# Fabstir/fabstir-vectordb

Measured on AMD Instinct MI355X. Metric: k-NN queries/sec at recall@10>=0.95, 1Mx384 f32, higher is better.
Workload: dtype f32

## Files before the change

fabstir-vectordb_amd/csrc/fvdb_graph.cpp:

```cpp
#include <algorithm>
#include <chrono>
#include <cstdio>
#include <cstdlib>
#include <cstring>
#include <map>
#include <new>
#include <string>
#include <vector>

#include "fvdb_internal.h"
#include "common.h"
#include "kernels_graph.h"
#include "kernels_graph_fast.h"
#include "kernels_graph_build.h"
#include "kernels_graph_maint.h"

using namespace fvdb;

struct fvdb_graph {
  fvdb_store* store = nullptr;
  uint32_t M = 0, M0 = 0;
  uint32_t stride0 = 0, strideU = 0;
  uint32_t n = 0, n_cap = 0;
  uint32_t u_rows = 0, u_cap = 0;
// ... 871 lines not shown
  if (mask && mask->stamp != g->mutations) FAIL(ctx, FVDB_E_INVALID, "stale mask: the graph changed after the mask was created");
  if (on && on->device != s->ctx->device) FAIL(ctx, FVDB_E_INVALID, "context of another device");
  if (s->d != s->dpad && slot != 0) FAIL(ctx, FVDB_E_UNSUPPORTED, "padded dimensions use slot 0 only");
  if (!g->uploaded || !g->has_entry) FAIL(ctx, FVDB_E_INVALID, "graph not uploaded");
  if (k == 0 || ef == 0 || ef > 4096) FAIL(ctx, FVDB_E_UNSUPPORTED, "ef must be in 1..4096");
  if (B == 0) return FVDB_OK;
  HIPCHK(ctx, hipSetDevice(ctx->device));
  std::lock_guard<std::mutex> lk(g->mu);
  const float* qd = q_dev;
  if (s->d != s->dpad) {
    HIPCHK(ctx, g->s_q.ensure((size_t)B * s->dpad * 4));
    hipLaunchKernelGGL(graph_pad_rows_kernel, dim3(cdiv((uint64_t)B * s->dpad, 256)), dim3(256), 0, ctx->stream, q_dev, s->d,
                       s->dpad, (uint64_t)B, g->s_q.as<float>());
    qd = g->s_q.as<float>();
  }
  SearchPlan sp{};
  int rc;
  if ((rc = search_scratch(g, ctx, slot, B, ef, &sp)) || (rc = search_kernel(g, ctx, ef, &sp))) return rc;
  if (sp.lds > 48 * 1024)
    HIPCHK(ctx, hipFuncSetAttribute(sp.fast ? (const void*)sp.fast : (const void*)sp.exact, hipFuncAttributeMaxDynamicSharedMemorySize, (int)sp.lds));
  if (!g->d_counters.p) {
    HIPCHK(ctx, g->d_counters.ensure(32));
    HIPCHK(ctx, hipMemsetAsync(g->d_counters.p, 0, 32, ctx->stream));
  }
  const uint32_t* deleted = mask ? mask->flags.as<uint32_t>() : g->d_deleted.as<uint32_t>();
  const uint32_t any_deleted = mask ? 1u : (g->n_deleted ? 1u : 0u);
  const GraphView gv{s->data, g->d_level.as<uint32_t>(), deleted, g->d_adj0.as<uint32_t>(), g->d_ubase.as<uint32_t>(),
                     g->d_adjU.as<uint32_t>(), g->stride0, g->strideU, g->n, s->dpad, g->entry, g->top_level, any_deleted,
                     g->d_counters.as<unsigned long long>(), graph_stamps_report(g)};
  hipEvent_t* ev = nullptr;
  if (s->ctx->profiling) {
    ev = g->kev[g->kev_n & 63];
    if (!ev[0]) {
      (void)hipEventCreate(&ev[0]);
      (void)hipEventCreate(&ev[1]);
    }
    (void)hipEventRecord(ev[0], ctx->stream);
  }
  if (sp.fast)
    hipLaunchKernelGGL(sp.fast, dim3(cdiv(B, 4)), dim3(256), sp.lds, ctx->stream, gv, qd, B, k, ef, sp.cand_cap, sp.wave_lds,
                       g->s_visited[slot].as<uint8_t>(), sp.vstride, sp.words, g->s_touched[slot].as<uint32_t>(), sp.tcap, out_nodes_dev,
                       out_dist_dev, out_counts_dev, out_status_dev, (HItem*)g->s_spill[slot].p, sp.spill_cap);
  else
    hipLaunchKernelGGL(sp.exact, dim3(B), dim3(64), sp.lds, ctx->stream, gv, qd, B, k, ef, sp.cand_cap, g->s_visited[slot].as<uint32_t>(),
                       sp.vstride / 4, g->s_touched[slot].as<uint32_t>(), sp.tcap, out_nodes_dev, out_dist_dev, out_counts_dev,
                       out_status_dev, sp.rh ? (HItem*)g->s_spill[slot].p : nullptr, sp.rh ? sp.spill_cap : 0u);
// ... 333 lines not shown
```

fabstir-vectordb_amd/host/capi.cpp:

```cpp
#include <cstring>
#include <new>

#include "fvdb_host.hpp"

using namespace fvdbh;

extern "C" {

void* fvh_ivf_new(fvdb_ctx* ctx, uint32_t n_clusters, uint32_t n_probe, uint32_t train_size, uint32_t max_iterations,
                  uint64_t seed) {
  IVFConfig c;
  c.n_clusters = n_clusters;
  c.n_probe = n_probe;
  c.train_size = train_size;
  c.max_iterations = max_iterations;
  c.seed = seed;
  if (!c.is_valid()) return nullptr;
  return new (std::nothrow) IVFIndex(ctx, c);
}
void fvh_ivf_free(void* p) { delete (IVFIndex*)p; }
int fvh_ivf_train(void* p, const float* x, uint64_t n, uint32_t d, fvdb_train_result* out) {
  return ((IVFIndex*)p)->train(x, n, d, out);
}
int fvh_ivf_set_trained(void* p, const float* c, uint32_t d) { return ((IVFIndex*)p)->set_trained(c, d); }
// ... 302 lines not shown
uint64_t fvh_hnsw_vacuum(void* p) { return ((HNSWIndex*)p)->vacuum(); }
int fvh_hnsw_vacuum_ex(void* p, uint64_t* removed) { return ((HNSWIndex*)p)->vacuum(removed); }
void fvh_hnsw_set_resident_vacuum(void* p, int on) { ((HNSWIndex*)p)->set_resident_vacuum(on != 0); }
int fvh_hnsw_resident_vacuum(void* p) { return ((HNSWIndex*)p)->resident_vacuum(); }
void fvh_hnsw_set_vacuum_keep_rows(void* p, int on) { ((HNSWIndex*)p)->set_vacuum_keep_rows(on != 0); }
int fvh_hnsw_vacuum_info(void* p, fvdb_graph_maintenance_info_t* out) { return ((HNSWIndex*)p)->vacuum_info(out); }
uint64_t fvh_hnsw_store_rows(void* p) { return ((HNSWIndex*)p)->store_rows(); }
int fvh_hybrid_get_vectors(void* p, const uint64_t* ids, uint64_t n, float* out, uint8_t* found) {
  return ((HybridIndex*)p)->get_vectors(ids, n, out, found);
}
void fvh_hybrid_set_resident_migration(void* p, int on) { ((HybridIndex*)p)->set_resident_migration(on != 0); }
int fvh_hybrid_migration_info(void* p, fvdb_maintenance_info_t* out) { return ((HybridIndex*)p)->migration_info(out); }
uint64_t fvh_hybrid_timestamp_count(void* p) { return ((HybridIndex*)p)->timestamp_count(); }
void fvh_hybrid_export_timestamps(void* p, uint64_t* ids, double* ts) { ((HybridIndex*)p)->export_timestamps(ids, ts); }
uint64_t fvh_hybrid_recent_count(void* p) { return ((HybridIndex*)p)->recent_count(); }
uint64_t fvh_hybrid_historical_count(void* p) { return ((HybridIndex*)p)->historical_count(); }
int fvh_hybrid_is_initialized(void* p) { return ((HybridIndex*)p)->is_initialized(); }
int fvh_hybrid_is_ivf_trained(void* p) { return ((HybridIndex*)p)->is_ivf_trained(); }
void* fvh_hybrid_hnsw(void* p) { return &((HybridIndex*)p)->recent(); }
void fvh_hybrid_set_sequential_graph(void* p, int on) { ((HybridIndex*)p)->set_sequential_graph(on != 0); }
int fvh_hybrid_sequential_graph(void* p) { return ((HybridIndex*)p)->sequential_graph(); }
double fvh_hybrid_recent_build_seconds(void* p) { return ((HybridIndex*)p)->recent_build_seconds(); }
void fvh_hybrid_set_blocking_writers(void* p, int on) { ((HybridIndex*)p)->set_blocking_writers(on != 0); }
int fvh_hybrid_blocking_writers(void* p) { return ((HybridIndex*)p)->blocking_writers(); }
void* fvh_hybrid_ivf(void* p) { return &((HybridIndex*)p)->historical(); }

}
```

fabstir-vectordb_amd/host/fvdb_host.hpp:

```cpp
#pragma once
#include <atomic>
#include <condition_variable>
#include <cstdint>
#include <memory>
#include <mutex>
#include <shared_mutex>
#include <string>
#include <unordered_map>
#include <unordered_set>
#include <vector>

#include "../../include/fvdb.h"

namespace fvdbh {

struct SplitMix64 {
  uint64_t s;
  explicit SplitMix64(uint64_t seed) : s(seed) {}
  uint64_t next() {
    uint64_t z = (s += 0x9E3779B97F4A7C15ull);
    z = (z ^ (z >> 30)) * 0xBF58476D1CE4E5B9ull;
    z = (z ^ (z >> 27)) * 0x94D049BB133111EBull;
    return z ^ (z >> 31);
  }
// ... 41 lines not shown
  int reserve(fvdb_ctx* c, uint64_t bytes, bool pinned) {
    if (bytes <= cap) return FVDB_OK;
    release();
    ctx = c;
    if (fvdb_dev_alloc(c, bytes, &dev) || (pinned && fvdb_host_alloc(c, bytes, &host))) return FVDB_E_OOM;
    cap = bytes;
    return FVDB_OK;
  }
  void release() {
    if (dev) fvdb_dev_free(ctx, dev);
    if (host) fvdb_host_free(ctx, host);
    dev = host = nullptr;
    cap = 0;
  }
};

typedef std::shared_ptr<fvdb_mask> MaskRef;
inline MaskRef adopt_mask(fvdb_mask* m) { return MaskRef(m, [](fvdb_mask* p) { fvdb_mask_destroy(p); }); }
inline bool mask_fresh(const MaskRef& m) {
  fvdb_mask_info_t info;
  return m && fvdb_mask_info(m.get(), &info) == FVDB_OK && !info.stale;
}

inline int slot_ctx(fvdb_ctx* base, bool borrow, fvdb_ctx** ctx) {
  if (*ctx) return FVDB_OK;
  if (!borrow) return fvdb_ctx_create(fvdb_ctx_device(base), ctx);
  *ctx = base;
  return FVDB_OK;
}

struct IVFConfig {
  uint32_t n_clusters = 256, n_probe = 16, train_size = 10000, max_iterations = 25;
  uint64_t seed = 0;
  bool is_valid() const { return n_clusters > 0 && n_probe > 0 && n_probe <= n_clusters && train_size > 0 && max_iterations > 0; }
};

class IVFIndex {
 public:
  IVFIndex(fvdb_ctx* ctx, const IVFConfig& cfg);
  ~IVFIndex();
  const IVFConfig& config() const { return cfg_; }
  bool is_trained() const { return trained_; }
  uint32_t dimension() const { return dim_; }
  uint64_t total_vectors() const { return total_; }
  int train(const float* data, uint64_t n, uint32_t dim, fvdb_train_result* out);
  int set_trained(const float* centroids, uint32_t dim);
  int get_centroids(float* out) const;
  int insert(uint64_t id, const float* v, uint32_t dim);
  int batch_insert(const uint64_t* ids, const float* v, uint64_t n, uint32_t dim, uint64_t* n_ok, int* first_error);
  int batch_insert_assigned(const uint64_t* ids, const float* v, uint64_t n, uint32_t dim, const uint32_t* clusters,
                            uint64_t* n_ok, int* first_error);
  int batch_insert_from_store(const uint64_t* ids, fvdb_store* store, const uint32_t* rows, uint64_t n, uint64_t* n_ok,
// ... 83 lines not shown
  uint64_t node_count() const { return n_registered_; }
  bool entry_point(uint64_t* id) const;
  uint32_t dimension() const { return dim_; }
  size_t assign_level();
  int insert(uint64_t id, const float* v, uint32_t dim, int64_t forced_level);
  int batch_insert(const uint64_t* ids, const float* v, uint64_t n, uint32_t dim, const int64_t* levels, uint64_t* n_ok,
                   int* first_error);
  void set_device_insert(bool on, int mode = 0) {
    device_insert_ = on;
    insert_mode_ = mode;
  }
  bool device_insert() const { return device_insert_; }
  int set_insert_visited(int mode, uint32_t table_slots = 0);
  int insert_info(fvdb_graph_insert_info_t* out);
  const fvdb_graph_insert_stats& insert_stats() const { return insert_stats_; }
  uint64_t host_path_inserts() const { return n_host_inserts_; }
  uint64_t graph_upload_bytes() const { return graph_ ? fvdb_graph_upload_bytes(graph_) : 0; }
  fvdb_graph* device_graph() { return sync_graph() == FVDB_OK ? graph_ : nullptr; }
  int search(const float* q, uint32_t B, uint32_t dim, uint32_t k, uint32_t ef, uint64_t* ids, float* dist,
             uint32_t* counts);
  int search_dev(const float* q_dev, uint32_t B, uint32_t dim, uint32_t k, uint32_t ef, uint64_t* ids, float* dist,
                 uint32_t* counts);
  static constexpr uint32_t kSlots = 16;
  bool search_dev_begin(const float* q_dev, uint32_t B, uint32_t dim, uint32_t k, uint32_t ef, int* rc, uint32_t slot = 0,
                        const AllowView* view = nullptr);
  int search_dev_end(const float* q_dev, uint32_t B, uint32_t dim, uint32_t k, uint32_t ef, uint64_t* ids, float* dist,
                     uint32_t* counts, uint32_t slot = 0, const AllowView* view = nullptr);
  int allowed_view(const uint64_t* allowed, uint64_t n_allowed, ViewRef* out);
  int search_allowed(const float* q, uint32_t B, uint32_t dim, uint32_t k, uint32_t ef, const uint64_t* allowed,
                     uint64_t n_allowed, uint64_t* ids, float* dist, uint32_t* counts);
  int search_dev_view(const float* q_dev, uint32_t B, uint32_t dim, uint32_t k, uint32_t ef, const AllowView& view,
                      uint64_t* ids, float* dist, uint32_t* counts);
  void set_scan_cutoff(uint64_t nodes) { scan_cutoff_ = nodes; }
  uint64_t scan_cutoff() const { return scan_cutoff_; }
  bool scans(const AllowView& v, uint32_t k) const { return v.allowed_live <= scan_cutoff_ && k <= FVDB_MAX_K; }
  uint64_t mask_builds() const { return mask_builds_; }
  int mark_deleted(uint64_t id);
  bool is_deleted(uint64_t id) const;
  uint64_t active_count() const;
  int vacuum(uint64_t* removed);
  uint64_t vacuum() {
    uint64_t r = 0;
    return vacuum(&r) == FVDB_OK ? r : 0;
  }
  void set_resident_vacuum(bool on) { resident_vacuum_ = on; }
  bool resident_vacuum() const { return resident_vacuum_; }
// ... 76 lines not shown
  bool resident_vacuum_ = true, vacuum_keep_rows_ = false;
  int vacuum_path_ = VACUUM_NONE;
  fvdb_graph_maintenance_info_t vacuum_info_{};
  uint64_t vacuum_host(const std::vector<uint8_t>& dead, uint64_t removed);
  void vacuum_adopt(bool reclaimed, const std::vector<uint8_t>& dead);
  bool host_link_reported_ = false;
  fvdb_graph_insert_stats insert_stats_{};
  uint64_t n_host_inserts_ = 0;
  void add_insert_stats(const fvdb_graph_insert_stats& st);
  int ensure_graph_handle();
  int ensure_host_graph();
  bool device_insert_ok() const;
  int check_insert(uint64_t id, const float* v, uint32_t dim) const;
  int insert_host(uint64_t id, const float* v, uint32_t dim, int64_t forced_level);
  int append_nodes(const uint64_t* ids, const uint32_t* levels, const float* v, uint32_t m, uint32_t* first);
  template <class L>
  int adopt_nodes(const uint64_t* ids, const float* v, uint64_t n, uint32_t dim, const L* levels);
  int link_and_publish(uint32_t row, bool on_device);
  int link_host(uint32_t row, std::vector<std::pair<uint32_t, uint32_t>>* touched);
  void finalize_insert(uint32_t row);
  struct DevSlot {
    fvdb_ctx* ctx = nullptr;
    DevBuf buf;
  };
  DevSlot slots_[kSlots];
  DevBuf d_q_;
  std::atomic<uint64_t> n_fallback_{0};
  std::mutex sync_mu_, walk_mu_, search_mu_;
  uint64_t scan_cutoff_ = 8192;
  std::mutex view_mu_;
  std::vector<uint64_t> view_key_;
  ViewRef view_;
  uint64_t mask_builds_ = 0;

  fvdb_ctx* ctx_;
  HNSWConfig cfg_;
  SplitMix64 rng_;
  fvdb_store* store_ = nullptr;
  uint32_t dim_ = 0;
  bool has_dim_ = false, has_entry_ = false, entry_lost_ = false;
  uint32_t entry_ = 0;
  uint64_t n_registered_ = 0;
  std::vector<uint64_t> ids_;
  std::vector<uint32_t> level_;
  std::vector<uint8_t> deleted_, registered_;
  std::vector<std::vector<std::vector<uint32_t>>> nbrs_;
  std::unordered_map<uint64_t, uint32_t> index_of_;
  std::vector<float> host_vecs_;
// ... 20 lines not shown
struct HybridSearchConfig {
  bool search_recent = true, search_historical = true;
  uint64_t recent_k = 0, historical_k = 0;
  uint64_t k = 10, hnsw_ef = 50, ivf_n_probe = 10;
};

class HybridIndex {
 public:
  HybridIndex(fvdb_ctx* ctx_ivf, fvdb_ctx* ctx_hnsw, const HybridConfig& cfg);
  ~HybridIndex();
  bool is_initialized() const { return initialized_; }
  bool is_ivf_trained() const { return ivf_trained_; }
  int initialize(const float* data, uint64_t n, uint32_t dim);
  int set_ivf_centroids(const float* c, uint32_t dim);
  int insert_with_timestamp(uint64_t id, const float* v, uint32_t dim, double ts, double now, int64_t level);
  int search(const float* q, uint32_t B, uint32_t dim, const HybridSearchConfig& cfg, double now, uint64_t* ids,
             float* dist, uint32_t* counts);
  int search_dev(const float* q_dev, uint32_t B, uint32_t dim, const HybridSearchConfig& cfg, double now,
                 uint64_t* ids, float* dist, uint32_t* counts);
  static constexpr uint32_t kSlots = HNSWIndex::kSlots;
  int search_dev_begin(uint32_t slot, const float* q_dev, uint32_t B, uint32_t dim, const HybridSearchConfig& cfg,
                       double now);
  int search_dev_end(uint32_t slot, uint64_t* ids, float* dist, uint32_t* counts);
  int attach_comm(fvdb_comm* comm);
  int search_sharded_begin(uint32_t slot, const float* q_dev, uint32_t B, uint32_t dim, const HybridSearchConfig& cfg,
                           int mode, double now = 0.0);
  int search_sharded_end(uint32_t slot, uint64_t* ids, float* dist, uint32_t* counts) {
    return search_dev_end(slot, ids, dist, counts);
  }
  uint32_t sharded_rows(uint32_t B, int mode) const;
  typedef int (*FilterFn)(uint64_t id, void* user);
  int search_with_filter(const float* q, uint32_t B, uint32_t dim, uint64_t k, FilterFn matches, void* user, double now,
                         uint64_t* ids, float* dist, uint32_t* counts);
  int search_allowed(const float* q, uint32_t B, uint32_t dim, const HybridSearchConfig& cfg, const uint64_t* allowed,
                     uint64_t n_allowed, double now, uint64_t* ids, float* dist, uint32_t* counts);
  void set_blocking_writers(bool on) { writers_wait_ = on; }
  bool blocking_writers() const { return writers_wait_; }
  bool busy() const {
    std::lock_guard<std::mutex> lk(slot_mu_);
    for (const Slot& s : slots_)
      if (s.active) return true;
    return false;
  }
  bool migration_due(double threshold_s, double now) const {
    return !pending_migration_.empty() && age_of(now, pending_min_ts_) >= threshold_s;
  }
// ... 43 lines not shown
                 std::vector<uint64_t>& hid, std::vector<float>& hv);
  bool sequential_graph_ = true;
  bool resident_migration_ = true;
  int migration_path_ = MIGRATION_NONE;
  fvdb_maintenance_info_t migration_info_{};
  std::atomic<bool> writers_wait_{false};
  int write_lock(std::unique_lock<std::shared_mutex>& w);
  double recent_build_s_ = 0.0;
  fvdb_comm* comm_ = nullptr;
  fvdb_sharded* sharded_ = nullptr;
  uint32_t shard_rank_ = 0, shard_world_ = 0;
  std::vector<uint32_t> shard_owner_;
  std::vector<uint64_t> shard_sizes_;
  uint64_t migrate_locked(double threshold_s, double now);
  bool busy_unlocked() const {
    for (const Slot& s : slots_)
      if (s.active) return true;
    return false;
  }
  mutable std::shared_mutex rw_;
  mutable std::mutex slot_mu_;
  std::condition_variable slot_cv_;
  fvdb_ctx* ctx_ivf_;
  struct Slot {
    DevBuf ivf;
    uint32_t ivf_rows = 0;
    fvdb_event* ivf_done = nullptr;
    fvdb_ctx* ivf_ctx = nullptr;
    bool active = false, ivf_in_flight = false, hnsw_in_flight = false, recent = false;
    DevBuf d_q;
    const float* q = nullptr;
    uint32_t B = 0, dim = 0, k = 0, rk = 0, hk = 0, ef = 0;
    MaskRef ivf_mask;
    HNSWIndex::ViewRef view;
  };
  Slot slots_[kSlots];
  struct Lease {
    static constexpr uint32_t kAnyFree = ~0u;
    enum How { kTake, kAdopt };
    Lease(HybridIndex* h, uint32_t slot, How how);
    ~Lease();
    Lease(const Lease&) = delete;
    Lease& operator=(const Lease&) = delete;
    void hand_over() { sl = nullptr; }
    uint32_t index() const { return (uint32_t)(sl - h->slots_); }
    HybridIndex* h;
// ... 24 lines not shown
```

fabstir-vectordb_amd/host/hnsw_index.cpp:

```cpp
#include <omp.h>

#include <algorithm>
#include <chrono>
#include <cstdio>
#include <cstdlib>
#include <cstring>

#include "fvdb_host.hpp"

namespace fvdbh {

void RustHeap::sift_up(size_t start, size_t pos) {
  Cand elt = data[pos];
  while (pos > start) {
    size_t parent = (pos - 1) / 2;
    if (le(elt, data[parent])) break;
    data[pos] = data[parent];
    pos = parent;
  }
  data[pos] = elt;
}
void RustHeap::push(Cand c) {
  size_t old = data.size();
  data.push_back(c);
// ... 77 lines not shown
  long quota = -1, period = -1;
  if (FILE* f = fopen("/sys/fs/cgroup/cpu.max", "r")) {
    char q[64];
    if (fscanf(f, "%63s %ld", q, &period) == 2 && strcmp(q, "max") != 0) quota = atol(q);
    fclose(f);
  } else if (FILE* f1 = fopen("/sys/fs/cgroup/cpu/cpu.cfs_quota_us", "r")) {
    if (fscanf(f1, "%ld", &quota) != 1) quota = -1;
    fclose(f1);
    if (FILE* f2 = fopen("/sys/fs/cgroup/cpu/cpu.cfs_period_us", "r")) {
      if (fscanf(f2, "%ld", &period) != 1) period = -1;
      fclose(f2);
    }
  }
  if (quota > 0 && period > 0) n = std::min<long>(n, std::max<long>(1, (quota + period - 1) / period));
  return std::max(1, std::min(n, 64));
}

static inline bool set_insert(std::vector<uint32_t>& s, uint32_t v) {
  if (std::find(s.begin(), s.end(), v) != s.end()) return false;
  s.push_back(v);
  return true;
}

HNSWIndex::HNSWIndex(fvdb_ctx* ctx, const HNSWConfig& cfg) : ctx_(ctx), cfg_(cfg), rng_(cfg.seed) {}

HNSWIndex::~HNSWIndex() {
  view_.reset();
  if (graph_) fvdb_graph_destroy(graph_);
  for (uint32_t i = 0; i < kSlots; ++i) {
    slots_[i].buf.release();
    if (i > 0 && slots_[i].ctx) fvdb_ctx_destroy(slots_[i].ctx);
  }
  d_q_.release();
  for (Walk* w : {&search_walk_, &insert_walk_})
    if (w->sc) fvdb_scorer_destroy(w->sc);
  if (store_) fvdb_store_destroy(store_);
}

bool HNSWIndex::entry_point(uint64_t* id) const {
  if (!has_entry_) return false;
  *id = ids_[entry_];
  return true;
}

size_t HNSWIndex::assign_level() {
  size_t level = 0;
  while (rng_.gen_f64() < 0.408) level += 1;
  return level;
}

int HNSWIndex::ensure_store(uint32_t dim) {
  if (store_) return FVDB_OK;
  return fvdb_store_create(ctx_, dim, 1024, &store_);
}
// ... 247 lines not shown

namespace {
struct WalkBlock {
  uint32_t* nodes;
  float* dist;
  uint32_t *counts, *status;
  uint64_t bytes;
  WalkBlock(void* base, uint32_t B, uint32_t k) {
    const uint64_t need = (uint64_t)B * std::max<uint32_t>(k, 1);
    nodes = (uint32_t*)base;
    dist = (float*)base + need;
    counts = (uint32_t*)base + 2 * need;
    status = counts + B;
    bytes = (2 * need + 2 * (uint64_t)B) * 4;
  }
};
}

int HNSWIndex::device_launch(const float* q_dev, uint32_t B, uint32_t k, uint32_t ef, uint32_t slot, const AllowView* view) {
  if (slot >= kSlots) return FVDB_E_INVALID;
  int rc = sync_graph();
  if (rc) return rc;
  DevSlot& sl = slots_[slot];
  rc = slot_ctx(ctx_, slot == 0, &sl.ctx);
  if (rc) return rc;
  const uint64_t bytes = WalkBlock(nullptr, B, k).bytes;
  rc = sl.buf.reserve(sl.ctx, bytes, true);
  if (rc) return rc;
  const WalkBlock d(sl.buf.dev, B, k);
  fvdb_ctx* on = slot == 0 ? nullptr : sl.ctx;
  if (!view)
    rc = fvdb_graph_search_dev_slot(graph_, on, slot, q_dev, B, k, ef, d.nodes, d.dist, d.counts, d.status);
  else if (scans(*view, k))
    rc = fvdb_graph_scan_allowed_dev_slot(graph_, on, slot, view->mask.get(), q_dev, B, k, d.nodes, d.dist, d.counts);
  else
    rc = fvdb_graph_search_dev_slot_masked(graph_, on, slot, view->mask.get(), q_dev, B, k, ef, d.nodes, d.dist, d.counts,
                                           d.status);
  if (!rc) rc = fvdb_dev_download_async(sl.ctx, sl.buf.host, sl.buf.dev, (size_t)bytes);
  return rc;
}

int HNSWIndex::device_collect(uint32_t B, uint32_t k, uint64_t* ids, float* dist, uint32_t* counts,
                              std::vector<uint32_t>& failed, uint32_t slot, bool scanned) {
  DevSlot& sl = slots_[slot];
  int rc = fvdb_ctx_synchronize(sl.ctx);
  if (rc) return rc;
  const WalkBlock h(sl.buf.host, B, k);
  std::memcpy(dist, h.dist, (size_t)B * k * 4);
  std::memcpy(counts, h.counts, (size_t)B * 4);
  for (uint32_t b = 0; b < B; ++b) {
    if (!scanned && h.status[b]) {
      failed.push_back(b);
      counts[b] = 0;
      continue;
    }
    for (uint32_t i = 0; i < k; ++i) {
      const uint32_t nd = h.nodes[(size_t)b * k + i];
      ids[(size_t)b * k + i] = i < counts[b] ? ids_[nd] : FVDB_NO_ID;
    }
  }
  return FVDB_OK;
}

int HNSWIndex::finish_failed(const float* q, bool q_on_device, uint32_t dim, uint32_t k, uint32_t ef, uint64_t* ids,
                             float* dist, uint32_t* counts, const std::vector<uint32_t>& failed, const AllowView* view) {
  if (failed.empty()) return FVDB_OK;
  n_fallback_ += failed.size();
  int rcg = ensure_host_graph();
// ... 743 lines not shown
```

fabstir-vectordb_amd/host/hybrid_index.cpp:

```cpp
#include <algorithm>
#include <chrono>
#include <cmath>
#include <cstdio>
#include <cstdlib>
#include <cstring>

#include "fvdb_host.hpp"

namespace fvdbh {

HybridIndex::HybridIndex(fvdb_ctx* ctx_ivf, fvdb_ctx* ctx_hnsw, const HybridConfig& cfg) : ctx_ivf_(ctx_ivf), cfg_(cfg) {
  recent_ = new HNSWIndex(ctx_hnsw, cfg.hnsw);
  historical_ = new IVFIndex(ctx_ivf, cfg.ivf);
}

HybridIndex::~HybridIndex() {
  for (Slot& sl : slots_) {
    sl.ivf.release();
    if (sl.ivf_done) fvdb_event_destroy(sl.ivf_done);
    sl.d_q.release();
    if (sl.ivf_ctx && sl.ivf_ctx != ctx_ivf_) fvdb_ctx_destroy(sl.ivf_ctx);
  }
  if (sharded_) fvdb_sharded_destroy(sharded_);
  delete recent_;
  delete historical_;
}

int HybridIndex::initialize(const float* data, uint64_t n, uint32_t dim) {
  if (n < cfg_.min_ivf_training_size) {
    ivf_trained_ = false;
    initialized_ = true;
    return FVDB_OK;
  }
  int rc = historical_->train(data, n, dim, nullptr);
  if (rc) return rc;
  historical_->clear_lists();
  ivf_trained_ = true;
  initialized_ = true;
  return FVDB_OK;
}

int HybridIndex::set_ivf_centroids(const float* c, uint32_t dim) {
  int rc = historical_->set_trained(c, dim);
  if (rc) return rc;
// ... 476 lines not shown
  return begin_explicit(slot, q_dev, B, dim, cfg, mode, now);
}

namespace {
struct IvfBlock {
  uint64_t* ids = nullptr;
  float* dist = nullptr;
  uint32_t* counts = nullptr;
  static uint64_t bytes(uint32_t rows, uint32_t hk) { return (uint64_t)rows * hk * 12 + (uint64_t)rows * 4; }
  IvfBlock() = default;
  IvfBlock(void* base, uint32_t rows, uint32_t hk) {
    const uint64_t need = (uint64_t)rows * hk;
    ids = (uint64_t*)base;
    dist = (float*)((char*)base + need * 8);
    counts = (uint32_t*)((char*)base + need * 12);
  }
};
}

int HybridIndex::begin_impl(uint32_t slot, const float* q_dev, uint32_t B, uint32_t dim, const HybridSearchConfig& cfg,
                            int shard_mode) {
  Slot& sl = slots_[slot];
  sl.ivf_in_flight = sl.hnsw_in_flight = false;
  const float* q_own = q_dev;
  uint32_t Bown = B, ivf_rows = B;
  if (shard_mode == FVDB_SHARD_STRONG) {
    const Slice s = strong_slice(B);
    q_own = q_dev + (size_t)s.lo * dim;
    Bown = s.hi - s.lo;
    ivf_rows = s.per;
  }
  const uint32_t B_ivf_in = B;
  B = Bown;
  sl.q = q_own;
  sl.B = B;
  sl.dim = dim;
  sl.k = (uint32_t)cfg.k;
  sl.rk = (uint32_t)(cfg.recent_k > 0 ? cfg.recent_k : cfg.k);
  sl.hk = (uint32_t)(cfg.historical_k > 0 ? cfg.historical_k : cfg.k);
  sl.ef = (uint32_t)cfg.hnsw_ef;
  sl.recent = cfg.search_recent;
  if (!initialized_ || sl.k == 0 || (B == 0 && shard_mode < 0)) return FVDB_OK;
  if (cfg.search_recent && B > 0) {
    int rcb = 0;
    sl.hnsw_in_flight = recent_->search_dev_begin(q_own, B, dim, sl.rk, sl.ef, &rcb, slot, sl.view.get());
  }
  if (cfg.search_historical && ivf_trained_) {
    const uint64_t bytes = IvfBlock::bytes(ivf_rows, sl.hk);
    if (int rc = sl.ivf.reserve(ctx_ivf_, bytes, true)) return rc;
    sl.ivf_rows = ivf_rows;
    const IvfBlock d(sl.ivf.dev, ivf_rows, sl.hk);
    static const bool one_stream = getenv("FVDB_IVF_ONE_STREAM") != nullptr;
    if (slot_ctx(ctx_ivf_, slot == 0 || one_stream, &sl.ivf_ctx)) return FVDB_E_HIP;
    fvdb_ctx* on = sl.ivf_ctx == ctx_ivf_ ? nullptr : sl.ivf_ctx;
    if (!sl.ivf_done && fvdb_event_create(sl.ivf_ctx, &sl.ivf_done)) return FVDB_E_HIP;
    if (shard_mode >= 0) {
      if (dim != historical_->dimension()) return FVDB_E_DIM;
      const int rcs = fvdb_ivf_search_sharded_begin(sharded_, on, on ? slot : 0, q_dev, B_ivf_in, sl.hk,
                                                    (uint32_t)cfg.ivf_n_probe, shard_mode, d.ids, d.dist, d.counts);
      if (rcs) return rcs;
      sl.ivf_in_flight = true;
    } else {
      const int rch = sl.ivf_mask ? historical_->search_dev_masked(sl.ivf_mask, q_dev, B, dim, sl.hk, (uint32_t)cfg.ivf_n_probe,
                                                                   d.ids, d.dist, d.counts, on, on ? slot : 0)
                                  : historical_->search_dev(q_dev, B, dim, sl.hk, (uint32_t)cfg.ivf_n_probe, d.ids, d.dist,
                                                            d.counts, on, on ? slot : 0);
      if (rch) return rch;
      sl.ivf_in_flight = true;
    }
    if (sl.ivf_in_flight) {
      if (fvdb_dev_download_async(sl.ivf_ctx, sl.ivf.host, sl.ivf.dev, (size_t)bytes) || fvdb_event_record(sl.ivf_ctx, sl.ivf_done))
        return FVDB_E_HIP;
    }
  }
  return FVDB_OK;
}

int HybridIndex::search_dev_end(uint32_t slot, uint64_t* ids, float* dist, uint32_t* counts) {
  if (slot >= kSlots) return FVDB_E_INVALID;
  Lease lease(this, slot, Lease::kAdopt);
  if (!lease.sl) return FVDB_E_INVALID;
  Slot& sl = *lease.sl;
  const uint32_t B = sl.B, k = sl.k;
  struct DropMasks {
    Slot& sl;
    ~DropMasks() {
      sl.ivf_mask.reset();
      sl.view.reset();
    }
// ... 46 lines not shown
  if (masked) {
    if (cfg.search_recent)
      if (int rc = recent_->allowed_view(allowed, n_allowed, &view)) return rc;
    if (cfg.search_historical && ivf_trained_)
      if (int rc = historical_->allowed_mask(allowed, n_allowed, &ivf_mask)) return rc;
  }
  Lease lease(this, Lease::kAnyFree, Lease::kTake);
  Slot& sl = *lease.sl;
  const uint32_t slot = lease.index();
  sl.ivf_mask = ivf_mask;
  sl.view = view;
  struct DropMasks {
    Slot* sl;
    ~DropMasks() {
      if (!sl) return;
      sl->ivf_mask.reset();
      sl->view.reset();
    }
  } drop_masks{&sl};
  const float* qd = q;
  if (!q_on_device) {
    const uint64_t bytes = (uint64_t)B * dim * 4;
    if (int rc = sl.d_q.reserve(ctx_ivf_, bytes, false)) return rc;
    if (slot_ctx(ctx_ivf_, slot == 0, &sl.ivf_ctx)) return FVDB_E_HIP;
    for (uint64_t i = 0; i < (uint64_t)B * dim; ++i)
      if (!(q[i] - q[i] == 0.0f)) return FVDB_E_NONFINITE;
    const int rcu = fvdb_dev_upload(sl.ivf_ctx, sl.d_q.dev, q, bytes);
    if (rcu) return rcu;
    qd = (const float*)sl.d_q.dev;
  }
  const int rc0 = begin_impl(slot, qd, B, dim, cfg);
  if (rc0 && !sl.hnsw_in_flight && !sl.ivf_in_flight) return rc0;
  lease.hand_over();
  drop_masks.sl = nullptr;
  if (rc0) {
    std::vector<uint64_t> ti((size_t)B * k);
    std::vector<float> td((size_t)B * k);
    std::vector<uint32_t> tc(B);
    (void)search_dev_end(slot, ti.data(), td.data(), tc.data());
    return rc0;
  }
  return search_dev_end(slot, ids, dist, counts);
}

int HybridIndex::search_allowed(const float* q, uint32_t B, uint32_t dim, const HybridSearchConfig& cfg, const uint64_t* allowed,
                                uint64_t n_allowed, double now, uint64_t* ids, float* dist, uint32_t* counts) {
  if (sharded_ || shard_world_) return FVDB_E_UNSUPPORTED;
// ... 45 lines not shown
```

fabstir-vectordb_amd/index.py:

```python
import ctypes as C
import os

import numpy as np

from . import _capi
from ._capi import f32p, u32p, u64p
from .engine import (STATUS_TO_EXC, DimensionMismatch, FvdbError, InconsistentDimensions,
                     InsufficientTrainingData, InvalidConfig, _f32, _ptr)

_HERE = os.path.dirname(os.path.abspath(__file__))
HOST_LIB_PATH = os.path.join(_capi.LIB_DIR, "libfvdb_host.so")
_host = None
i64p = C.POINTER(C.c_int64)
f64p = C.POINTER(C.c_double)
vp, u64, u32, i32, i64, dbl = C.c_void_p, C.c_uint64, C.c_uint32, C.c_int, C.c_int64, C.c_double

HOST_SIGNATURES = {
    "fvh_ivf_new": (vp, [vp, u32, u32, u32, u32, u64]),
    "fvh_ivf_free": (None, [vp]),
    "fvh_ivf_train": (i32, [vp, f32p, u64, u32, C.POINTER(_capi.TrainResult)]),
    "fvh_ivf_set_trained": (i32, [vp, f32p, u32]),
    "fvh_ivf_get_centroids": (i32, [vp, f32p]),
    "fvh_ivf_is_trained": (i32, [vp]),
    "fvh_ivf_dimension": (u32, [vp]),
# ... 80 lines not shown
    "fvh_hybrid_delete": (i32, [vp, u64, dbl]),
    "fvh_hybrid_migrate": (u64, [vp, dbl, dbl]),
    "fvh_hybrid_vacuum": (i32, [vp, u64p, u64p]),
    "fvh_ivf_vacuum": (i32, [vp, u64p]),
    "fvh_hnsw_vacuum": (u64, [vp]),
    "fvh_hnsw_vacuum_ex": (i32, [vp, u64p]),
    "fvh_hnsw_set_resident_vacuum": (None, [vp, i32]),
    "fvh_hnsw_resident_vacuum": (i32, [vp]),
    "fvh_hnsw_set_vacuum_keep_rows": (None, [vp, i32]),
    "fvh_hnsw_vacuum_info": (i32, [vp, vp]),
    "fvh_hnsw_store_rows": (u64, [vp]),
    "fvh_hybrid_from_parts": (i32, [vp, u64p, f64p, u64, u64, u64, i32]),
    "fvh_hybrid_timestamp_count": (u64, [vp]),
    "fvh_hybrid_export_timestamps": (None, [vp, u64p, f64p]),
    "fvh_hybrid_recent_count": (u64, [vp]),
    "fvh_hybrid_historical_count": (u64, [vp]),
    "fvh_hybrid_is_initialized": (i32, [vp]),
    "fvh_hybrid_is_ivf_trained": (i32, [vp]),
    "fvh_hybrid_hnsw": (vp, [vp]),
    "fvh_hybrid_set_sequential_graph": (None, [vp, i32]),
    "fvh_hybrid_sequential_graph": (i32, [vp]),
    "fvh_hybrid_recent_build_seconds": (dbl, [vp]),
    "fvh_hybrid_set_blocking_writers": (None, [vp, i32]),
    "fvh_hybrid_blocking_writers": (i32, [vp]),
    "fvh_hybrid_ivf": (vp, [vp]),
    "fvh_ivf_get_vectors": (i32, [vp, u64p, u64, f32p, C.POINTER(C.c_uint8)]),
    "fvh_hybrid_get_vectors": (i32, [vp, u64p, u64, f32p, C.POINTER(C.c_uint8)]),
    "fvh_hybrid_set_resident_migration": (None, [vp, i32]),
    "fvh_hybrid_migration_info": (i32, [vp, vp]),
}


def load_host():
    global _host
    if _host is not None:
        return _host
    _capi.load()
    if not os.path.exists(HOST_LIB_PATH):
        raise ImportError(f"{HOST_LIB_PATH} not found: build it with `make -C fabstir-vectordb_amd`")
    lib = C.CDLL(HOST_LIB_PATH)
    for name, (res, args) in HOST_SIGNATURES.items():
        fn = getattr(lib, name)
        fn.restype = res
        fn.argtypes = args
    _host = lib
    return lib
# ... 513 lines not shown
            x = x.reshape(len(training_data), -1)
        self._check(self.lib.fvh_hybrid_initialize(self.h, _ptr(x, f32p), x.shape[0], x.shape[1]))

    def set_ivf_centroids(self, centroids):
        c = _rows(centroids)
        self._check(self.lib.fvh_hybrid_set_ivf_centroids(self.h, _ptr(c, f32p), c.shape[1]))

    def insert_with_timestamp(self, id, vector, timestamp, now, level=-1):
        v = _f32(vector).reshape(-1)
        self._check(self.lib.fvh_hybrid_insert(self.h, int(id), _ptr(v, f32p), v.size, float(timestamp), float(now), level))

    def insert(self, id, vector, now=0.0, level=-1):
        self.insert_with_timestamp(id, vector, now, now, level)

    def set_sequential_graph(self, on):
        self.lib.fvh_hybrid_set_sequential_graph(self.h, int(bool(on)))

    def sequential_graph(self):
        return bool(self.lib.fvh_hybrid_sequential_graph(self.h))

    def set_blocking_writers(self, on):
        self.lib.fvh_hybrid_set_blocking_writers(self.h, int(bool(on)))

    def recent_build_seconds(self):
        return float(self.lib.fvh_hybrid_recent_build_seconds(self.h))

    def bulk_insert(self, ids, vectors, timestamps, now):
        v = _rows(vectors)
        ids = np.ascontiguousarray(ids, np.uint64)
        ts = np.ascontiguousarray(timestamps, np.float64)
        self._check(self.lib.fvh_hybrid_bulk_insert(self.h, _ptr(ids, u64p), _ptr(v, f32p), v.shape[0], v.shape[1],
                                                    _ptr(ts, f64p), float(now)))

    def bulk_insert_sharded(self, ids, vectors, timestamps, now, rank, world):
        v = _rows(vectors)
        ids = np.ascontiguousarray(ids, np.uint64)
        ts = np.ascontiguousarray(timestamps, np.float64)
        owner = np.zeros(self.n_clusters, np.uint32)
        self._check(self.lib.fvh_hybrid_bulk_insert_sharded(self.h, _ptr(ids, u64p), _ptr(v, f32p), v.shape[0],
                                                            v.shape[1], _ptr(ts, f64p), float(now), rank, world,
                                                            _ptr(owner, u32p)))
        return owner

    def search(self, queries, k, now=0.0, hnsw_ef=50, ivf_n_probe=10, search_recent=True, search_historical=True,
               recent_k=0, historical_k=0):
        return self._search(self.lib.fvh_hybrid_search, queries, k, hnsw_ef, ivf_n_probe, int(search_recent),
# ... 151 lines not shown
```

Baseline: 1.677 million.

## Add configurable stream plan mapping search slots to shared role streams

Introduces a RoleStreams pool so HNSW traversal and IVF search slots map onto a configurable number of streams (env or API, optionally sized from hardware queue count). Per-slot completion now uses recorded events instead of whole-stream synchronize, so slots that share a stream can wait on only their own work. By default every slot still gets its own stream, which preserves the previous behaviour. It also adds a one-time stream synchronize after the counters memset.

Measured after the change: 1.664 million. About the same (-0.8%).

```diff
diff --git a/fabstir-vectordb_amd/csrc/fvdb_graph.cpp b/fabstir-vectordb_amd/csrc/fvdb_graph.cpp
--- a/fabstir-vectordb_amd/csrc/fvdb_graph.cpp
+++ b/fabstir-vectordb_amd/csrc/fvdb_graph.cpp
@@ -917,6 +917,7 @@
   if (!g->d_counters.p) {
     HIPCHK(ctx, g->d_counters.ensure(32));
     HIPCHK(ctx, hipMemsetAsync(g->d_counters.p, 0, 32, ctx->stream));
+    HIPCHK(ctx, hipStreamSynchronize(ctx->stream));
   }
   const uint32_t* deleted = mask ? mask->flags.as<uint32_t>() : g->d_deleted.as<uint32_t>();
   const uint32_t any_deleted = mask ? 1u : (g->n_deleted ? 1u : 0u);
diff --git a/fabstir-vectordb_amd/host/capi.cpp b/fabstir-vectordb_amd/host/capi.cpp
--- a/fabstir-vectordb_amd/host/capi.cpp
+++ b/fabstir-vectordb_amd/host/capi.cpp
@@ -348,6 +348,8 @@
 int fvh_hybrid_sequential_graph(void* p) { return ((HybridIndex*)p)->sequential_graph(); }
 double fvh_hybrid_recent_build_seconds(void* p) { return ((HybridIndex*)p)->recent_build_seconds(); }
 void fvh_hybrid_set_blocking_writers(void* p, int on) { ((HybridIndex*)p)->set_blocking_writers(on != 0); }
+int fvh_hybrid_set_stream_plan(void* p, uint32_t T, uint32_t I) { return ((HybridIndex*)p)->set_stream_plan(T, I); }
+void fvh_hybrid_stream_plan(void* p, uint32_t* T, uint32_t* I) { ((HybridIndex*)p)->stream_plan(T, I); }
 int fvh_hybrid_blocking_writers(void* p) { return ((HybridIndex*)p)->blocking_writers(); }
 void* fvh_hybrid_ivf(void* p) { return &((HybridIndex*)p)->historical(); }
 
diff --git a/fabstir-vectordb_amd/host/fvdb_host.hpp b/fabstir-vectordb_amd/host/fvdb_host.hpp
--- a/fabstir-vectordb_amd/host/fvdb_host.hpp
+++ b/fabstir-vectordb_amd/host/fvdb_host.hpp
@@ -87,12 +87,43 @@
   return m && fvdb_mask_info(m.get(), &info) == FVDB_OK && !info.stale;
 }
 
-inline int slot_ctx(fvdb_ctx* base, bool borrow, fvdb_ctx** ctx) {
-  if (*ctx) return FVDB_OK;
-  if (!borrow) return fvdb_ctx_create(fvdb_ctx_device(base), ctx);
-  *ctx = base;
-  return FVDB_OK;
-}
+class RoleStreams {
+ public:
+  static constexpr uint32_t kMax = 16;
+  explicit RoleStreams(fvdb_ctx* base) : base_(base) {}
+  ~RoleStreams() {
+    for (uint32_t i = 1; i < kMax; ++i)
+      if (own_[i]) fvdb_ctx_destroy(own_[i]);
+  }
+  RoleStreams(const RoleStreams&) = delete;
+  RoleStreams& operator=(const RoleStreams&) = delete;
+  uint32_t count() const { return n_; }
+  void set_count(uint32_t n) { n_ = n < 1 ? 1 : (n > kMax ? kMax : n); }
+  int of_slot(uint32_t slot, fvdb_ctx** out) {
+    const uint32_t j = slot % n_;
+    if (j == 0) {
+      *out = base_;
+      return FVDB_OK;
+    }
+    std::lock_guard<std::mutex> lk(mu_);
+    if (!own_[j])
+      if (int rc = fvdb_ctx_create(fvdb_ctx_device(base_), &own_[j])) return rc;
+    *out = own_[j];
+    return FVDB_OK;
+  }
+  int create_all() {
+    fvdb_ctx* c;
+    for (uint32_t j = 1; j < n_; ++j)
+      if (int rc = of_slot(j, &c)) return rc;
+    return FVDB_OK;
+  }
+
+ private:
+  fvdb_ctx* base_;
+  fvdb_ctx* own_[kMax] = {};
+  uint32_t n_ = kMax;
+  std::mutex mu_;
+};
 
 struct IVFConfig {
   uint32_t n_clusters = 256, n_probe = 16, train_size = 10000, max_iterations = 25;
@@ -222,6 +253,11 @@
   int search_dev(const float* q_dev, uint32_t B, uint32_t dim, uint32_t k, uint32_t ef, uint64_t* ids, float* dist,
                  uint32_t* counts);
   static constexpr uint32_t kSlots = 16;
+  int set_traversal_streams(uint32_t n) {
+    streams_.set_count(n);
+    return n < kSlots ? streams_.create_all() : FVDB_OK;
+  }
+  uint32_t traversal_streams() const { return streams_.count(); }
   bool search_dev_begin(const float* q_dev, uint32_t B, uint32_t dim, uint32_t k, uint32_t ef, int* rc, uint32_t slot = 0,
                         const AllowView* view = nullptr);
   int search_dev_end(const float* q_dev, uint32_t B, uint32_t dim, uint32_t k, uint32_t ef, uint64_t* ids, float* dist,
@@ -344,8 +380,10 @@
   struct DevSlot {
     fvdb_ctx* ctx = nullptr;
     DevBuf buf;
+    fvdb_event* done = nullptr;
   };
   DevSlot slots_[kSlots];
+  RoleStreams streams_;
   DevBuf d_q_;
   std::atomic<uint64_t> n_fallback_{0};
   std::mutex sync_mu_, walk_mu_, search_mu_;
@@ -412,6 +450,9 @@
   int search_dev_begin(uint32_t slot, const float* q_dev, uint32_t B, uint32_t dim, const HybridSearchConfig& cfg,
                        double now);
   int search_dev_end(uint32_t slot, uint64_t* ids, float* dist, uint32_t* counts);
+  int set_stream_plan(uint32_t T, uint32_t I);
+  void stream_plan(uint32_t* T, uint32_t* I);
+  static void auto_plan(int hw_queues, uint32_t* T, uint32_t* I);
   int attach_comm(fvdb_comm* comm);
   int search_sharded_begin(uint32_t slot, const float* q_dev, uint32_t B, uint32_t dim, const HybridSearchConfig& cfg,
                            int mode, double now = 0.0);
@@ -501,6 +542,11 @@
   mutable std::mutex slot_mu_;
   std::condition_variable slot_cv_;
   fvdb_ctx* ctx_ivf_;
+  RoleStreams ivf_streams_;
+  uint32_t plan_T_ = 0, plan_I_ = 0;
+  bool plan_applied_ = false, plan_by_queues_ = false;
+  std::mutex plan_mu_;
+  int apply_stream_plan();
   struct Slot {
     DevBuf ivf;
     uint32_t ivf_rows = 0;
diff --git a/fabstir-vectordb_amd/host/hnsw_index.cpp b/fabstir-vectordb_amd/host/hnsw_index.cpp
--- a/fabstir-vectordb_amd/host/hnsw_index.cpp
+++ b/fabstir-vectordb_amd/host/hnsw_index.cpp
@@ -123,14 +123,14 @@
   return true;
 }
 
-HNSWIndex::HNSWIndex(fvdb_ctx* ctx, const HNSWConfig& cfg) : ctx_(ctx), cfg_(cfg), rng_(cfg.seed) {}
+HNSWIndex::HNSWIndex(fvdb_ctx* ctx, const HNSWConfig& cfg) : streams_(ctx), ctx_(ctx), cfg_(cfg), rng_(cfg.seed) {}
 
 HNSWIndex::~HNSWIndex() {
   view_.reset();
   if (graph_) fvdb_graph_destroy(graph_);
   for (uint32_t i = 0; i < kSlots; ++i) {
     slots_[i].buf.release();
-    if (i > 0 && slots_[i].ctx) fvdb_ctx_destroy(slots_[i].ctx);
+    if (slots_[i].done) fvdb_event_destroy(slots_[i].done);
   }
   d_q_.release();
   for (Walk* w : {&search_walk_, &insert_walk_})
@@ -424,13 +424,14 @@
   int rc = sync_graph();
   if (rc) return rc;
   DevSlot& sl = slots_[slot];
-  rc = slot_ctx(ctx_, slot == 0, &sl.ctx);
-  if (rc) return rc;
+  rc = streams_.of_slot(slot, &sl.ctx);
+  if (rc) return rc;
+  if (!sl.done && (rc = fvdb_event_create(ctx_, &sl.done))) return rc;
   const uint64_t bytes = WalkBlock(nullptr, B, k).bytes;
-  rc = sl.buf.reserve(sl.ctx, bytes, true);
+  rc = sl.buf.reserve(ctx_, bytes, true);
   if (rc) return rc;
   const WalkBlock d(sl.buf.dev, B, k);
-  fvdb_ctx* on = slot == 0 ? nullptr : sl.ctx;
+  fvdb_ctx* on = sl.ctx == ctx_ ? nullptr : sl.ctx;
   if (!view)
     rc = fvdb_graph_search_dev_slot(graph_, on, slot, q_dev, B, k, ef, d.nodes, d.dist, d.counts, d.status);
   else if (scans(*view, k))
@@ -439,13 +440,14 @@
     rc = fvdb_graph_search_dev_slot_masked(graph_, on, slot, view->mask.get(), q_dev, B, k, ef, d.nodes, d.dist, d.counts,
                                            d.status);
   if (!rc) rc = fvdb_dev_download_async(sl.ctx, sl.buf.host, sl.buf.dev, (size_t)bytes);
+  if (!rc) rc = fvdb_event_record(sl.ctx, sl.done);
   return rc;
 }
 
 int HNSWIndex::device_collect(uint32_t B, uint32_t k, uint64_t* ids, float* dist, uint32_t* counts,
                               std::vector<uint32_t>& failed, uint32_t slot, bool scanned) {
   DevSlot& sl = slots_[slot];
-  int rc = fvdb_ctx_synchronize(sl.ctx);
+  int rc = fvdb_event_wait(sl.ctx, sl.done);
   if (rc) return rc;
   const WalkBlock h(sl.buf.host, B, k);
   std::memcpy(dist, h.dist, (size_t)B * k * 4);
diff --git a/fabstir-vectordb_amd/host/hybrid_index.cpp b/fabstir-vectordb_amd/host/hybrid_index.cpp
--- a/fabstir-vectordb_amd/host/hybrid_index.cpp
+++ b/fabstir-vectordb_amd/host/hybrid_index.cpp
@@ -9,9 +9,65 @@
 
 namespace fvdbh {
 
-HybridIndex::HybridIndex(fvdb_ctx* ctx_ivf, fvdb_ctx* ctx_hnsw, const HybridConfig& cfg) : ctx_ivf_(ctx_ivf), cfg_(cfg) {
+HybridIndex::HybridIndex(fvdb_ctx* ctx_ivf, fvdb_ctx* ctx_hnsw, const HybridConfig& cfg)
+    : ctx_ivf_(ctx_ivf), ivf_streams_(ctx_ivf), cfg_(cfg) {
   recent_ = new HNSWIndex(ctx_hnsw, cfg.hnsw);
   historical_ = new IVFIndex(ctx_ivf, cfg.ivf);
+  if (const char* e = getenv("FVDB_STREAM_PLAN")) {
+    unsigned t = 0, i = 0;
+    if (sscanf(e, "%u,%u", &t, &i) == 2) (void)set_stream_plan(t, i);
+    else if (!strcmp(e, "queues")) plan_by_queues_ = true;
+  }
+}
+
+void HybridIndex::auto_plan(int hw_queues, uint32_t* T, uint32_t* I) {
+  if (hw_queues >= (int)(2 * kSlots)) {
+    *T = *I = kSlots;
+  } else if (hw_queues >= 6) {
+    *T = *I = (uint32_t)hw_queues / 2;
+  } else if (hw_queues >= 4) {
+    *T = 3;
+    *I = (uint32_t)hw_queues - 3;
+  } else {
+    *T = hw_queues >= 3 ? 2 : 1;
+    *I = 1;
+  }
+}
+
+int HybridIndex::set_stream_plan(uint32_t T, uint32_t I) {
+  if ((T == 0) != (I == 0) || T > kSlots || I > kSlots) return FVDB_E_INVALID;
+  std::unique_lock<std::shared_mutex> w(rw_);
+  if (busy()) return FVDB_E_INVALID;
+  std::lock_guard<std::mutex> lk(plan_mu_);
+  plan_T_ = T;
+  plan_I_ = I;
+  plan_applied_ = false;
+  return FVDB_OK;
+}
+
+int HybridIndex::apply_stream_plan() {
+  std::lock_guard<std::mutex> lk(plan_mu_);
+  if (plan_applied_) return FVDB_OK;
+  uint32_t T = plan_T_, I = plan_I_;
+  if (T == 0 && !plan_by_queues_) {
+    T = I = kSlots;
+  } else if (T == 0) {
+    fvdb_ctx_info_t info{};
+    if (fvdb_ctx_info(ctx_ivf_, &info)) return FVDB_E_HIP;
+    auto_plan(info.hw_queues, &T, &I);
+  }
+  if (int rc = recent_->set_traversal_streams(T)) return rc;
+  ivf_streams_.set_count(I);
+  if (I < kSlots)
+    if (int rc = ivf_streams_.create_all()) return rc;
+  plan_applied_ = true;
+  return FVDB_OK;
+}
+
+void HybridIndex::stream_plan(uint32_t* T, uint32_t* I) {
+  (void)apply_stream_plan();
+  *T = recent_->traversal_streams();
+  *I = ivf_streams_.count();
 }
 
 HybridIndex::~HybridIndex() {
@@ -19,7 +75,6 @@
     sl.ivf.release();
     if (sl.ivf_done) fvdb_event_destroy(sl.ivf_done);
     sl.d_q.release();
-    if (sl.ivf_ctx && sl.ivf_ctx != ctx_ivf_) fvdb_ctx_destroy(sl.ivf_ctx);
   }
   if (sharded_) fvdb_sharded_destroy(sharded_);
   delete recent_;
@@ -542,6 +597,7 @@
                             int shard_mode) {
   Slot& sl = slots_[slot];
   sl.ivf_in_flight = sl.hnsw_in_flight = false;
+  if (apply_stream_plan()) return FVDB_E_HIP;
   const float* q_own = q_dev;
   uint32_t Bown = B, ivf_rows = B;
   if (shard_mode == FVDB_SHARD_STRONG) {
@@ -570,21 +626,20 @@
     if (int rc = sl.ivf.reserve(ctx_ivf_, bytes, true)) return rc;
     sl.ivf_rows = ivf_rows;
     const IvfBlock d(sl.ivf.dev, ivf_rows, sl.hk);
-    static const bool one_stream = getenv("FVDB_IVF_ONE_STREAM") != nullptr;
-    if (slot_ctx(ctx_ivf_, slot == 0 || one_stream, &sl.ivf_ctx)) return FVDB_E_HIP;
+    if (ivf_streams_.of_slot(slot, &sl.ivf_ctx)) return FVDB_E_HIP;
     fvdb_ctx* on = sl.ivf_ctx == ctx_ivf_ ? nullptr : sl.ivf_ctx;
-    if (!sl.ivf_done && fvdb_event_create(sl.ivf_ctx, &sl.ivf_done)) return FVDB_E_HIP;
+    if (!sl.ivf_done && fvdb_event_create(ctx_ivf_, &sl.ivf_done)) return FVDB_E_HIP;
     if (shard_mode >= 0) {
       if (dim != historical_->dimension()) return FVDB_E_DIM;
-      const int rcs = fvdb_ivf_search_sharded_begin(sharded_, on, on ? slot : 0, q_dev, B_ivf_in, sl.hk,
+      const int rcs = fvdb_ivf_search_sharded_begin(sharded_, on, slot, q_dev, B_ivf_in, sl.hk,
                                                     (uint32_t)cfg.ivf_n_probe, shard_mode, d.ids, d.dist, d.counts);
       if (rcs) return rcs;
       sl.ivf_in_flight = true;
     } else {
       const int rch = sl.ivf_mask ? historical_->search_dev_masked(sl.ivf_mask, q_dev, B, dim, sl.hk, (uint32_t)cfg.ivf_n_probe,
-                                                                   d.ids, d.dist, d.counts, on, on ? slot : 0)
+                                                                   d.ids, d.dist, d.counts, on, slot)
                                   : historical_->search_dev(q_dev, B, dim, sl.hk, (uint32_t)cfg.ivf_n_probe, d.ids, d.dist,
-                                                            d.counts, on, on ? slot : 0);
+                                                            d.counts, on, slot);
       if (rch) return rch;
       sl.ivf_in_flight = true;
     }
@@ -677,7 +732,7 @@
   if (!q_on_device) {
     const uint64_t bytes = (uint64_t)B * dim * 4;
     if (int rc = sl.d_q.reserve(ctx_ivf_, bytes, false)) return rc;
-    if (slot_ctx(ctx_ivf_, slot == 0, &sl.ivf_ctx)) return FVDB_E_HIP;
+    if (apply_stream_plan() || ivf_streams_.of_slot(slot, &sl.ivf_ctx)) return FVDB_E_HIP;
     for (uint64_t i = 0; i < (uint64_t)B * dim; ++i)
       if (!(q[i] - q[i] == 0.0f)) return FVDB_E_NONFINITE;
     const int rcu = fvdb_dev_upload(sl.ivf_ctx, sl.d_q.dev, q, bytes);
diff --git a/fabstir-vectordb_amd/index.py b/fabstir-vectordb_amd/index.py
--- a/fabstir-vectordb_amd/index.py
+++ b/fabstir-vectordb_amd/index.py
@@ -126,6 +126,8 @@
     "fvh_hybrid_sequential_graph": (i32, [vp]),
     "fvh_hybrid_recent_build_seconds": (dbl, [vp]),
     "fvh_hybrid_set_blocking_writers": (None, [vp, i32]),
+    "fvh_hybrid_set_stream_plan": (i32, [vp, u32, u32]),
+    "fvh_hybrid_stream_plan": (None, [vp, u32p, u32p]),
     "fvh_hybrid_blocking_writers": (i32, [vp]),
     "fvh_hybrid_ivf": (vp, [vp]),
     "fvh_ivf_get_vectors": (i32, [vp, u64p, u64, f32p, C.POINTER(C.c_uint8)]),
@@ -685,6 +687,14 @@
     def set_blocking_writers(self, on):
         self.lib.fvh_hybrid_set_blocking_writers(self.h, int(bool(on)))
 
+    def set_stream_plan(self, traversal_streams=0, ivf_streams=0):
+        self._check(self.lib.fvh_hybrid_set_stream_plan(self.h, int(traversal_streams), int(ivf_streams)))
+
+    def stream_plan(self):
+        t, i = C.c_uint32(0), C.c_uint32(0)
+        self.lib.fvh_hybrid_stream_plan(self.h, C.byref(t), C.byref(i))
+        return int(t.value), int(i.value)
+
     def recent_build_seconds(self):
         return float(self.lib.fvh_hybrid_recent_build_seconds(self.h))
 
```
